# UCRajkumar/ecSeg

Measured on AMD Instinct MI355X. Metric: DAPI images/sec (1392x1040, 4-class metaseg), higher is better.
Workload: dtype f32; 1 GPU; BASELINE configs[1] + post-process: 16 synthetic 1040x1392 uint8 DAPI images per GPU per step, 35 tiles of 256x256 each, canonical U-Net base 64 (96.2 GFLOP/patch, seeded random weights) -> stitch/uint8-quantise/argmax -> meta_inference -> ecDNA count; unet_base=64, patches_per_image=35, parallelism=image-parallel x1, all-gather of 128-B records, allgather=none (1 rank)

## Files before the change

ecseg_amd/build.py:

```python
import os
import subprocess
import sys

HERE = os.path.dirname(os.path.abspath(__file__))
CSRC = os.path.join(HERE, 'csrc')
LIB = os.path.join(HERE, 'libecseg_hip.so')
SOURCES = ['api.hip', 'filter_layout.hip', 'model_load.hip', 'plan_run.hip', 'segment.hip', 'drivers.hip', 'unet_kernels.hip', 'layer_kernels.hip', 'wino4_kernel.hip', 'wino4s_kernel.hip', 'wino4r_kernel.hip', 'convs_kernel.hip', 'wino16_kernel.hip', 'post_kernels.hip', 'interseg_kernels.hip', 'fishdist_kernels.hip', 'fishspot_kernels.hip', 'host_codec.cpp', 'host_io.cpp', 'comm.hip']
EXTRA_FLAGS = {'wino4_kernel.hip': ['-fno-slp-vectorize'], 'wino4s_kernel.hip': ['-fno-slp-vectorize'], 'wino4r_kernel.hip': ['-fno-slp-vectorize']}
HEADERS = [os.path.join(CSRC, f) for f in ('common.h', 'ctx.h', 'device_util.h', 'wino4_consts.inc', 'wino4_region.inc', 'wino4_combine.inc', 'wino4_head.inc')] + \
    [os.path.join(HERE, '..', 'include', 'ecseg_hip.h')]


def source_hash():
    import hashlib
    h = hashlib.sha256()
    names = sorted(f for f in os.listdir(CSRC) if f.endswith(('.hip', '.h', '.inc')))
    for f in names:
        h.update(f.encode() + b'\0')
        with open(os.path.join(CSRC, f), 'rb') as fh:
            h.update(fh.read())
    return h.hexdigest()


def _hipcc():
    for c in (os.environ.get('HIPCC'), '/opt/rocm/bin/hipcc', 'hipcc'):
        if c and (os.path.isabs(c) and os.path.exists(c) or not os.path.isabs(c)):
            return c
    return 'hipcc'


def needs_build():
    if not os.path.exists(LIB):
        return True
    t = os.path.getmtime(LIB)
    deps = [os.path.join(CSRC, s) for s in SOURCES] + HEADERS
    return any(os.path.getmtime(d) > t for d in deps if os.path.exists(d))


def build(force=False, verbose=True):
    if not force and not needs_build():
        return LIB
    objs = []
    procs = []
    for s in SOURCES:
        obj = os.path.join(CSRC, os.path.splitext(s)[0] + '.o')
        cmd = [_hipcc(), '-O3', '-std=c++17', '--offload-arch=gfx950', '-fPIC', '-Wall', '-Wno-unused-function'] + \
            EXTRA_FLAGS.get(s, []) + ['-c', os.path.join(CSRC, s), '-o', obj]
        if verbose:
            print(' '.join(cmd), flush=True)
        procs.append((subprocess.Popen(cmd), cmd))
        objs.append(obj)
    for p, cmd in procs:
        if p.wait() != 0:
            raise RuntimeError('hipcc failed: ' + ' '.join(cmd))
    cmd = [_hipcc(), '--offload-arch=gfx950', '-shared', '-fPIC', '-o', LIB] + objs + ['-lz', '-ldl']
    if verbose:
        print(' '.join(cmd), flush=True)
    subprocess.check_call(cmd)
    return LIB


if __name__ == '__main__':
    build(force='--force' in sys.argv)
    print(LIB)
```

ecseg_amd/csrc/api.hip:

```cpp
#include <cstdio>
#include <cstdlib>
#include "ctx.h"

namespace ecseg {

namespace { std::string g_create_error; }

int fail(ecseg_ctx* h, int code, const std::string& msg) {
    if (h) h->err = msg; else g_create_error = msg;
    return code;
}
int fail_hip(ecseg_ctx* h, hipError_t e, const char* what) {
    return fail(h, ECSEG_E_HIP, std::string(what) + ": " + hipGetErrorString(e));
}

int check_model(ecseg_ctx* h) {
    if (!h) return ECSEG_E_INVALID;
    if (!h->has_model) return fail(h, ECSEG_E_NOMODEL, "no model loaded (call ecseg_model_load first)");
    return ECSEG_OK;
}

}

using namespace ecseg;

extern "C" {

int ecseg_abi_version(void) { return ECSEG_ABI_VERSION; }

int ecseg_create(ecseg_ctx** out, int device_id) {
    if (!out) return fail(nullptr, ECSEG_E_INVALID, "out is NULL");
    *out = nullptr;
    int ndev = 0;
    hipError_t e = hipGetDeviceCount(&ndev);
    if (e != hipSuccess || ndev <= 0) return fail(nullptr, ECSEG_E_HIP, std::string("no HIP device: ") + hipGetErrorString(e));
    if (device_id < 0 || device_id >= ndev) return fail(nullptr, ECSEG_E_INVALID, "device_id out of range");
    if ((e = hipSetDevice(device_id)) != hipSuccess) return fail_hip(nullptr, e, "hipSetDevice");
    if (!getenv("ECSEG_SPIN_WAIT") || atoi(getenv("ECSEG_SPIN_WAIT")) == 0) {
        if (hipSetDeviceFlags(hipDeviceScheduleBlockingSync) != hipSuccess) (void)hipGetLastError();
    }
    ecseg_ctx* h = new ecseg_ctx();
    h->device = device_id;
    hipDeviceProp_t prop;
    if (hipGetDeviceProperties(&prop, device_id) == hipSuccess) {
        snprintf(h->devname, sizeof(h->devname), "%s (%s)", prop.name, prop.gcnArchName);
    }
    if ((e = hipStreamCreateWithFlags(&h->stream, hipStreamNonBlocking)) != hipSuccess) {
        delete h;
        return fail_hip(nullptr, e, "hipStreamCreate");
    }
    if ((e = hipStreamCreateWithFlags(&h->stream2, hipStreamNonBlocking)) != hipSuccess) {
        (void)hipStreamDestroy(h->stream);
        delete h;
        return fail_hip(nullptr, e, "hipStreamCreate");
    }
    for (auto& ev : h->ev) (void)hipEventCreate(&ev);
    if (hipMalloc(reinterpret_cast<void**>(&h->zero_page), 1024) == hipSuccess) (void)hipMemset(h->zero_page, 0, 1024);
    else h->zero_page = nullptr;
    *out = h;
    return ECSEG_OK;
}

void ecseg_destroy(ecseg_ctx* h) {
    if (!h) return;
    (void)hipSetDevice(h->device);
    (void)hipStreamSynchronize(h->stream);
    (void)hipStreamSynchronize(h->stream2);
    free_model(h);
    if (h->zero_page) (void)hipFree(h->zero_page);
    { DevMem dying(std::move(static_cast<DevMem&>(*h))); }
    for (auto& ev : h->ev) if (ev) (void)hipEventDestroy(ev);
    if (h->ev_block) (void)hipEventDestroy(h->ev_block);
    if (h->stream_in) { (void)hipStreamSynchronize(h->stream_in); (void)hipStreamDestroy(h->stream_in); }
    if (h->ev_pre) (void)hipEventDestroy(h->ev_pre);
    for (hipEvent_t e : h->prof_events) (void)hipEventDestroy(e);
    for (hipEvent_t e : h->grp_events) (void)hipEventDestroy(e);
    for (hipEvent_t e : h->lane_events) (void)hipEventDestroy(e);
    for (hipStream_t ls : h->lane_streams) { (void)hipStreamSynchronize(ls); (void)hipStreamDestroy(ls); }
    (void)hipStreamDestroy(h->stream2);
    (void)hipStreamDestroy(h->stream);
    delete h;
}

const char* ecseg_last_error(ecseg_ctx* h) { return h ? h->err.c_str() : g_create_error.c_str(); }

int ecseg_device_name(ecseg_ctx* h, char* buf, int buflen) {
    if (!h || !buf || buflen <= 0) return ECSEG_E_INVALID;
    snprintf(buf, buflen, "%s", h->devname);
    return ECSEG_OK;
}

void* ecseg_stream(ecseg_ctx* h) { return h ? (void*)h->stream : nullptr; }

int ecseg_set_images_per_group(ecseg_ctx* h, int n) {
    if (!h || n < 0) return ECSEG_E_INVALID;
    h->images_per_group = n;
    return ECSEG_OK;
}

int ecseg_set_option(ecseg_ctx* h, const char* key, int value) {
    if (!h || !key) return ECSEG_E_INVALID;
    const std::string k(key);
    if (k == "overlap_post") h->overlap_post = value != 0;
    else if (k == "blocking_wait") h->blocking_wait = value != 0;
    else if (k == "fuse_pool") h->fuse_pool = value != 0;
    else if (k == "fuse_head") h->fuse_head = value != 0;
    else if (k == "wino_resident") h->wino_resident = value != 0;
    else if (k == "wino16") h->wino16 = value != 0;
    else if (k == "fuse_first") h->fuse_first = value != 0;
    else if (k == "wino4_split") h->wino4_split = value != 0;
    else if (k == "crop") h->crop = value != 0;
    else if (k == "winograd") {
        h->use_winograd = value < 0 ? 0 : value > 3 ? 3 : (int)value;
        return ensure_split_images(h);
    }
    else if (k == "post_chunk" && value >= 1) h->post_chunk = value;
    else if (k == "images_per_group" && value >= 0) h->images_per_group = value;
    else if (k == "crop_mask") h->crop_mask = value != 0;
    else if (k == "unet_lanes" && value >= 0 && value <= 8) h->unet_lanes = value;
    else if (k == "lane_auto_windows" && value >= 0) h->lane_auto_windows = value;
    else return fail(h, ECSEG_E_INVALID, "unknown option or bad value: " + k);
    return ECSEG_OK;
}

int ecseg_host_alloc(ecseg_ctx* h, size_t bytes, void** out) {
    if (!h || !out) return ECSEG_E_INVALID;
    *out = nullptr;
    if (bytes == 0) return ECSEG_OK;
    if (hipSetDevice(h->device) != hipSuccess) { (void)hipGetLastError(); return ECSEG_E_HIP; }
    const hipError_t e = hipHostMalloc(out, bytes, hipHostMallocPortable);
    if (e != hipSuccess) { (void)hipGetLastError(); *out = nullptr; return e == hipErrorOutOfMemory ? ECSEG_E_NOMEM : ECSEG_E_HIP; }
    return ECSEG_OK;
}

int ecseg_host_free(ecseg_ctx* h, void* p) {
    if (!h) return ECSEG_E_INVALID;
    if (!p) return ECSEG_OK;
    if (hipSetDevice(h->device) != hipSuccess || hipHostFree(p) != hipSuccess) { (void)hipGetLastError(); return ECSEG_E_HIP; }
    return ECSEG_OK;
}

int ecseg_get_timings(ecseg_ctx* h, float* ms_out) {
    if (!h || !ms_out) return ECSEG_E_INVALID;
    for (int k = 0; k < ECSEG_T_N; ++k) ms_out[k] = h->stage_ms[k];
    return ECSEG_OK;
}

int ecseg_set_kernel_profiling(ecseg_ctx* h, int enabled) {
    if (!h) return ECSEG_E_INVALID;
    h->profile_kernels = enabled != 0;
    return ECSEG_OK;
}

int ecseg_get_conv_profile(ecseg_ctx* h, double* total_ms, int64_t* launches, double* flops) {
    if (!h) return ECSEG_E_INVALID;
    if (total_ms) *total_ms = h->last_conv_ms;
    if (launches) *launches = h->last_conv_launches;
    if (flops) *flops = h->last_conv_flops;
    return ECSEG_OK;
}

int ecseg_debug_peek(ecseg_ctx* h, float* out, int n) {
#ifdef ECSEG_DIAG
    if (!h || !out || n < 0 || n > 240 || !h->zero_page) return ECSEG_E_INVALID;
    HIP_TRY(h, hipSetDevice(h->device));
    HIP_TRY(h, hipMemcpy(out, h->zero_page + 16, (size_t)n * sizeof(float), hipMemcpyDeviceToHost));
    return ECSEG_OK;
#else
    (void)out; (void)n;
    return fail(h, ECSEG_E_UNSUPPORTED, "ecseg_debug_peek: the shipped library carries no diagnostic kernels (build with -DECSEG_DIAG)");
#endif
}

int ecseg_get_conv_launch_profile(ecseg_ctx* h, int max_records, int32_t* op_index, int32_t* kind, float* ms, double* flops,
                                  double* executed_flops) {
    if (!h || max_records < 0) return ECSEG_E_INVALID;
    const int n = (int)std::min<size_t>(h->prof_recs.size(), (size_t)max_records);
    for (int k = 0; k < n; ++k) {
        const ecseg_ctx::ProfRec& r = h->prof_recs[k];
        if (op_index) op_index[k] = r.op;
        if (kind) kind[k] = r.kind;
        if (ms) ms[k] = r.ms;
        if (flops) flops[k] = r.flops;
        if (executed_flops) executed_flops[k] = r.exec_flops;
    }
    return n;
}

int ecseg_get_conv_executed_flops(ecseg_ctx* h, double* flops) {
    if (!h || !flops) return ECSEG_E_INVALID;
    *flops = h->last_conv_exec_flops;
    return ECSEG_OK;
}

}
```

ecseg_amd/csrc/common.h:

```cpp
#pragma once
#include <hip/hip_runtime.h>
#include <stdint.h>

#include "../../include/ecseg_hip.h"

namespace ecseg {

struct TView {
    float* p;
    int h, w, c, cs;
};

struct ConvParams {
    TView in, out;
    const float* wt;
    const float* bias;
    int n;
    int R, S;
    int pad_top, pad_left;
    int act;
    float alpha;
    int cin_chunks;
    int coutp;
    int convt;
    int kT, crop_top, crop_left;
    int convt_ext;
    int phase_a, phase_b;
    int tap_zero_mask;
    int stride;
    const float* zero;
    TView pool;
    const float* head_w; const float* head_b; TView head_out; int head_k, head_act, head_only;
    const int32_t* lut; int lut_len, per_image;
    const int32_t* in_box; int box_first;
    int force_tw;
    int resident;
    int w4_split;
    const float* first_w; const float* first_b; int first_act; float first_alpha;
    long wt_chunk_stride, wt_tap_stride;
};

#ifndef ECSEG_W4_PA
#define ECSEG_W4_PA 0.625
#define ECSEG_W4_PB 1.5
#endif
constexpr double W4_PA = ECSEG_W4_PA, W4_PB = ECSEG_W4_PB;

inline long wt_chunk_pitch(int np_total) { return (long)2 * np_total * 4 + 32; }
inline long wt_tap_pitch(int np_total, int chunks) { return wt_chunk_pitch(np_total) * chunks + 96; }

hipError_t launch_conv_mfma(const ConvParams& p, hipStream_t s);
bool       conv_mfma_supported(const ConvParams& p);
int        conv_mfma_ntile(int cout);
hipError_t launch_conv_wino(const ConvParams& p, hipStream_t s);
int        conv_wino_ntile(int cout);
hipError_t launch_conv_wino16(const ConvParams& p, hipStream_t s);
bool       conv_wino16_supported(const ConvParams& p);
bool       conv_wino16_first_supported(const ConvParams& p);
hipError_t launch_conv_wino4(const ConvParams& p, hipStream_t s);
bool       conv_wino4_supported(const ConvParams& p);
bool       conv_wino4_span_ok(const ConvParams& p, int windows);
hipError_t launch_conv_wino4r(const ConvParams& p, hipStream_t s);
bool       conv_wino4r_supported(const ConvParams& p);
hipError_t launch_conv_wino4s(const ConvParams& p, hipStream_t s);
bool       conv_wino4s_supported(const ConvParams& p);
size_t     wino4s_image_bytes(int cin, int cout);
hipError_t launch_wino4s_filter(const float* wt_wino4, void* dst, int cin, int cout, hipStream_t s);
hipError_t launch_convs(const ConvParams& p, hipStream_t s);
bool       convs_supported(const ConvParams& p);
size_t     convs_image_bytes(int cin, int np);
hipError_t launch_convs_filter(const float* wt_fp32, void* dst, int cin, int np, hipStream_t s);

hipError_t launch_conv_small_cin(const TView& in, const TView& out, const float* w_hwio, const float* bias, int n,
                                 int R, int S, int pad_top, int pad_left, int act, float alpha, hipStream_t s);
hipError_t launch_conv_head(const TView& in, const TView& out, const float* w_io, const float* bias, int n, int act,
                            float alpha, hipStream_t s);
hipError_t launch_conv_generic(const TView& in, const TView& out, const float* w_hwio, const float* bias, int n,
                               int R, int S, int stride, int pad_top, int pad_left, int act, float alpha, hipStream_t s);
hipError_t launch_convt_generic(const TView& in, const TView& out, const float* w_hwoi, const float* bias, int n,
                                int R, int S, int stride, int crop_top, int crop_left, int act, float alpha,
                                hipStream_t s);
hipError_t launch_maxpool(const TView& in, const TView& out, int n, int kh, int kw, int stride, int mode, hipStream_t s);
hipError_t launch_global_pool(const TView& in, const TView& out, int n, int mode, hipStream_t s);
hipError_t launch_upsample(const TView& in, const TView& out, int n, int factor, int mode, hipStream_t s);
hipError_t launch_affine(const TView& in, const TView& out, const float* scale, const float* shift, int n, int act,
                         float alpha, hipStream_t s);
hipError_t launch_add(const TView& a, const TView& b, const TView& out, int n, int act, float alpha, hipStream_t s);
hipError_t launch_copy(const TView& in, const TView& out, int n, int off_y, int off_x, hipStream_t s);
hipError_t launch_softmax(const TView& in, const TView& out, int n, hipStream_t s);
hipError_t launch_u8_to_f32(const uint8_t* in, float* out, size_t count, hipStream_t s);

hipError_t launch_conv_mfma_tap(const ConvParams& p, int dilation, hipStream_t s);
bool       conv_mfma_tap_supported(const ConvParams& p);
hipError_t launch_conv_generic_dil(const TView& in, const TView& out, const float* w_hwio, const float* bias, int n, int R, int S,
                                   int stride, int stride_x, int dilation, int dilation_x, int pad_top, int pad_left, int act, float alpha,
                                   hipStream_t s);
hipError_t launch_dwconv(const TView& in, const TView& out, const float* w, const float* bias, int n, int kh, int kw, int stride,
                         int dilation, int pad_top, int pad_left, int mult, int act, float alpha, hipStream_t s);
hipError_t launch_binary(const TView& a, const TView& b, const TView& out, int n, int mode, int act, float alpha, hipStream_t s);
hipError_t launch_prelu(const TView& in, const TView& out, const float* slope, int n, int per_element, hipStream_t s);
hipError_t launch_layernorm(const TView& in, const TView& out, const float* gamma, const float* beta, int n, float eps, hipStream_t s);
hipError_t launch_pool_pad(const TView& in, const TView& out, int n, int kh, int kw, int stride, int pad_top, int pad_left, int mode,
                           hipStream_t s);
hipError_t launch_tile_patches(const uint8_t* gray, int n_img, int H, int W, const int32_t* pos_yx, int n_pos,
                               float* out, hipStream_t s);

hipError_t launch_stitch_argmax(const float* probs, int prob_cs, const int32_t* src_map, int n_img, int n_pos,
                                int H, int W, uint8_t* labels, hipStream_t s, int32_t* tie_risk = nullptr, int32_t* tie_shards = nullptr);
hipError_t launch_stitch_probs(const float* probs, int prob_cs, const int32_t* src_map, int n_img, int n_pos,
                               int H, int W, float* out, hipStream_t s);

struct PostWorkspace {
    int32_t* L;
    uint32_t* area;
    unsigned long long* sumy;
    unsigned long long* sumx;
    uint32_t* flag;
    uint8_t* tmpA;
    uint8_t* tmpB;
    int32_t* list;
    int32_t* g;
    uint8_t* tile_any;
    uint32_t* own_bits;
    double* binned;
    int32_t* binstart;
    size_t binned_cap;
    int cap_img;
    size_t cap_px;
};
enum { G_STRIDE = 32, G_SHARDS = 16 };
enum { G_SLOTS = 6 };
enum { NUCLEUS_BIN_EXTENT = 32768 };

hipError_t run_meta_inference(PostWorkspace& ws, uint8_t* img, int n_img, int H, int W, int32_t* n_ec_dev,
                              hipStream_t s);
hipError_t run_count_cc(PostWorkspace& ws, const uint8_t* mask, int n_img, int H, int W, int32_t* n_dev,
                        long long* px_dev, hipStream_t s);
hipError_t run_ccl_labels(PostWorkspace& ws, const uint8_t* mask, int n_img, int H, int W, int conn,
                          int32_t* labels_dev, hipStream_t s);
hipError_t run_count_coloc(PostWorkspace& ws, const uint8_t* ob1, const uint8_t* ob2, int n_img, int H, int W,
                           int32_t* n_dev, hipStream_t s);
hipError_t run_count_hsr(PostWorkspace& ws, const uint8_t* chrom, const uint8_t* fish, int n_img, int H, int W,
                         int thr, int32_t* n_dev, hipStream_t s);
hipError_t run_overlay(PostWorkspace& ws, const uint8_t* labels, const uint8_t* rgb, int n_img, int H, int W, int C,
                       int sens, int hsr_thr, long long* out_dev, hipStream_t s);
hipError_t launch_u16_to_u8(const uint16_t* in, uint8_t* out, size_t count, hipStream_t s);
hipError_t run_preprocess(const void* img, int n_img, int H, int W, int C, int bps, uint8_t* gray, int32_t* inverted,
                          uint32_t* hist_ws, hipStream_t s);

struct RegionBufs { int32_t* rid; int32_t* blk; int32_t* misc; unsigned long long* acc; int32_t* bb; int64_t* rec; int cap; };
hipError_t run_nuclei_regions(const uint8_t* seg, const uint8_t* img, int H, int W, int img_w, int C, int ch0, int32_t* labels,
                              const RegionBufs& b, hipStream_t s);
hipError_t run_nucleus_crops(const int32_t* labels, const uint8_t* img, int W, int img_w, int C, const int32_t* desc, int n,
                             const int order[3], uint8_t* out, int32_t* chmax, hipStream_t s);

struct FishDistBufs { int32_t* rid; int32_t* par; int32_t* blk; int32_t* misc; int2* flist; int2* clist; unsigned* acc; int32_t* val;
                      int32_t* off; int32_t* cur; int64_t* rec; unsigned long long* pbest; int32_t* proots; };
int fishdist_slices(int n);
hipError_t run_fishdist_cells(const int32_t* labels, int H, int W, const FishDistBufs& b, hipStream_t s);
hipError_t run_fishdist_records(int32_t* labels, const uint8_t* lsq, int H, int W, int C, int fi, int ci, int n, const FishDistBufs& b,
                                hipStream_t s);

struct FishSpotBufs { int32_t* rid; int32_t* mx; uint8_t* thr; uint8_t* bnd; int32_t* par; int32_t* sz; unsigned long long* acc;
                      unsigned* cnt; int32_t* val; int64_t* rec; };
hipError_t run_fishspot(int32_t* labels, const uint8_t* img, int H, int W, int C, int np, const int ch[3], const double* wts, int K,
                        double normal_thr, const double ithr[3], int min_cc, int line_t, int n, const FishSpotBufs& b, hipStream_t s);

}
```

ecseg_amd/csrc/ctx.h:

```cpp
#pragma once
#include <algorithm>
#include <array>
#include <map>
#include <string>
#include <utility>
#include <vector>

#include "common.h"

namespace ecseg {

int fail(ecseg_ctx* h, int code, const std::string& msg);
int fail_hip(ecseg_ctx* h, hipError_t e, const char* what);
#define HIP_TRY(h, call) do { hipError_t _e = (call); if (_e != hipSuccess) return fail_hip((h), _e, #call); } while (0)

template <typename T>
struct DevBuf {
    T* p = nullptr;
    size_t cap = 0;
    DevBuf() = default;
    DevBuf(DevBuf&& o) noexcept { swap(o); }
    DevBuf(const DevBuf&) = delete;
    DevBuf& operator=(const DevBuf&) = delete;
    ~DevBuf() { if (p) (void)hipFree(p); }
    void swap(DevBuf& o) { std::swap(p, o.p); std::swap(cap, o.cap); }
    operator T*() const { return p; }
    int ensure(ecseg_ctx* h, size_t need_elems) {
        if (need_elems <= cap && p) return ECSEG_OK;
        if (p) { hipError_t e = hipFree(p); p = nullptr; cap = 0; if (e != hipSuccess) return fail_hip(h, e, "hipFree"); }
        if (need_elems == 0) need_elems = 1;
        hipError_t e = hipMalloc(reinterpret_cast<void**>(&p), need_elems * sizeof(T));
        if (e != hipSuccess) { p = nullptr; return fail(h, ECSEG_E_NOMEM, std::string("hipMalloc: ") + hipGetErrorString(e)); }
        cap = need_elems;
        return ECSEG_OK;
    }
};

struct OpRt {
    ecseg_op_desc d;
    int path;
    float* wt = nullptr;
    float* wt_wino = nullptr;
    float* wt_wino4 = nullptr;
    float* wt_wino16 = nullptr;
    void* wt_split1 = nullptr;
    int s1_cin = 0, s1_np = 0;
    void* wt_wino4s = nullptr;
    int w4_cin = 0, w4_cout = 0;
    int coutp_wino = 0;
    float* bias = nullptr;
    float* head_w4 = nullptr;
    float* head_b4 = nullptr;
    bool crop_ok = false;
    std::string crop_code;
    float* scale = nullptr;
    float* shift = nullptr;
    int cin_chunks = 0, coutp = 0;
    int subpixel = 0;
    float* ph_wt[4] = {nullptr, nullptr, nullptr, nullptr};
    int ph_R[4] = {0, 0, 0, 0}, ph_S[4] = {0, 0, 0, 0}, ph_pt[4] = {0, 0, 0, 0}, ph_pl[4] = {0, 0, 0, 0};
    double flops = 0.0;
};
enum { PATH_MFMA = 1, PATH_SMALL_CIN = 2, PATH_HEAD = 3, PATH_GENERIC = 4, PATH_OTHER = 5, PATH_TAP = 6  };

struct CropLut {
    DevBuf<int32_t> dev; int len = 0; int size = 0; std::vector<int> start;
};
struct StitchPlan {
    int n_pos = 0;
    DevBuf<int32_t> pos_dev;
    DevBuf<int32_t> map_dev;
    std::vector<int> box;
    std::map<std::string, CropLut> luts;
    std::map<std::string, DevBuf<int32_t>> boxes;
};

struct LaneSpec { int w0, cnt; hipStream_t s; };

void free_post_workspace(PostWorkspace& w);
struct OwnedPostWorkspace : PostWorkspace {
    OwnedPostWorkspace() : PostWorkspace{} {}
    OwnedPostWorkspace(OwnedPostWorkspace&& o) noexcept : PostWorkspace(o) { static_cast<PostWorkspace&>(o) = PostWorkspace{}; }
    ~OwnedPostWorkspace() { free_post_workspace(*this); }
};

struct DevMem {
    std::map<std::pair<int, int>, StitchPlan> stitch;
    DevBuf<uint8_t> d_gray, d_raw, d_post;
    DevBuf<int32_t> d_tie;
    DevBuf<int32_t> d_tie_sh;
    DevBuf<float> d_sprobs;
    DevBuf<uint8_t> d_aux8;
    DevBuf<uint8_t> d_pre;
    DevBuf<uint8_t> d_u8in;
    DevBuf<int32_t> d_i32;
    DevBuf<long long> d_i64;
    DevBuf<float> d_probs_in;
    DevBuf<uint32_t> d_hist;
    OwnedPostWorkspace ws;
    DevBuf<int32_t> d_iseg_lab, d_iseg_rid, d_iseg_blk, d_iseg_misc, d_iseg_bb, d_iseg_desc, d_iseg_max;
    DevBuf<uint8_t> d_iseg_img, d_iseg_crops;
    DevBuf<unsigned long long> d_iseg_acc;
    DevBuf<int64_t> d_iseg_rec;
    DevBuf<int32_t> d_fd_lab, d_fd_rid, d_fd_par, d_fd_blk, d_fd_misc, d_fd_val, d_fd_off, d_fd_cur, d_fd_proots;
    DevBuf<uint8_t> d_fd_lsq;
    DevBuf<int2> d_fd_flist, d_fd_clist;
    DevBuf<unsigned> d_fd_acc;
    DevBuf<int64_t> d_fd_rec;
    DevBuf<unsigned long long> d_fd_pbest;
    DevBuf<int32_t> d_fs_lab, d_fs_rid, d_fs_blk, d_fs_misc, d_fs_mx, d_fs_par, d_fs_sz, d_fs_val;
    DevBuf<uint8_t> d_fs_img, d_fs_thr, d_fs_bnd;
    DevBuf<double> d_fs_w;
    DevBuf<unsigned long long> d_fs_acc;
    DevBuf<unsigned> d_fs_cnt;
    DevBuf<int64_t> d_fs_rec;
};

}

struct ecseg_ctx : ecseg::DevMem {
    int device = 0;
    hipStream_t stream = nullptr;
    hipStream_t stream2 = nullptr;
    std::vector<hipStream_t> lane_streams;
    std::vector<hipEvent_t> lane_events;
    int unet_lanes = 0;
    int lane_auto_windows = 70;
    bool lanes_ok = false;
    std::string err;
    char devname[256] = {0};

    bool has_model = false;
    std::vector<ecseg_tensor_desc> tensors;
    std::vector<ecseg::OpRt> ops;
    int n_buffers = 0;
    std::vector<size_t> buf_floats;
    std::vector<float*> bufs;
    int cap_patches = 0;
    std::vector<float*> dev_allocs;
    float* zero_page = nullptr;
    int input_tensor = -1, output_tensor = -1;
    std::vector<int> consumers;
    double flops_per_patch = 0.0, mfma_flops_per_patch = 0.0;

    int images_per_group = 0;
    const void* pre_host = nullptr; size_t pre_bytes = 0;
    const void* next_host = nullptr; size_t next_bytes = 0;
    hipStream_t stream_in = nullptr;
    hipEvent_t ev_pre = nullptr;
    int iseg_H = 0, iseg_W = 0, iseg_img_w = 0, iseg_C = 0, iseg_n = -1;
    int post_chunk = 64;
    int overlap_post = 0;
    int blocking_wait = 1;
    hipEvent_t ev_block = nullptr;
    int fuse_pool = 1;
    int crop = 1;
    int crop_mask = 1;
    int fuse_head = 1;
    int use_winograd = 2;
    int wino4_split = 1;
    int wino16 = 1;
    int wino_resident = 1;
    int fuse_first = 1;

    hipEvent_t ev[ECSEG_T_N + 1] = {};
    float stage_ms[ECSEG_T_N] = {};
    bool profile_kernels = false;
    std::vector<hipEvent_t> prof_events;
    std::vector<hipEvent_t> grp_events;
    size_t prof_used = 0;
    double prof_flops = 0.0, prof_exec_flops = 0.0;
    struct ProfRec { int op; int kind; double flops, exec_flops; float ms; };
    std::vector<ProfRec> prof_recs;
    double last_conv_ms = 0.0; long long last_conv_launches = 0; double last_conv_flops = 0.0, last_conv_exec_flops = 0.0;
};

namespace ecseg {

inline TView view_of(const ecseg_ctx* h, int t) {
    const ecseg_tensor_desc& d = h->tensors[t];
    TView v;
    v.p = h->bufs[d.buffer] + d.c_offset;
    v.h = d.h; v.w = d.w; v.c = d.c; v.cs = d.c_stride;
    return v;
}

inline float stage_elapsed(hipEvent_t a, hipEvent_t b) {
    float t = 0.f;
    return hipEventElapsedTime(&t, a, b) == hipSuccess ? t : 0.f;
}

inline void drop_sent_ahead(ecseg_ctx* h) {
    h->next_host = nullptr; h->next_bytes = 0;
    h->pre_host = nullptr; h->pre_bytes = 0;
}

int check_model(ecseg_ctx* h);

std::vector<float> relayout_conv(const float* w, int R, int S, int cin, int cout, int chunks, int np);
std::vector<float> relayout_wino16(const std::vector<float>& u, int cin, int cout);
std::vector<float> winograd_filter(const float* w, int cin, int cout);
std::vector<float> winograd4_filter(const float* w, int cin, int cout);
std::vector<float> relayout_convt(const float* w, int kT, int cin, int cout, int chunks, int coutp);
std::vector<float> relayout_convt_subpixel(const float* w, int k, int cin, int cout, int chunks, int coutp);
struct PhaseFilter { std::vector<float> hwio; int R, S, pt, pl; };
std::array<PhaseFilter, 4> convt_phase_filters(const float* w, int k, int cin, int cout, int crop_top, int crop_left);

void free_model(ecseg_ctx* h);
int ensure_split_images(ecseg_ctx* h);

int ensure_patches(ecseg_ctx* h, int n);
int windows_per_group(const ecseg_ctx* h);
int run_plan(ecseg_ctx* h, int n_all, StitchPlan* crop = nullptr, const std::vector<LaneSpec>* lanes = nullptr);
void prof_begin(ecseg_ctx* h);
void prof_end(ecseg_ctx* h);

int get_stitch(ecseg_ctx* h, int H, int W, StitchPlan** out);
int ensure_post(ecseg_ctx* h, int n_img, size_t px);

}
```

ecseg_amd/csrc/plan_run.hip:

```cpp
#include "ctx.h"

namespace ecseg {

int ensure_patches(ecseg_ctx* h, int n) {
    if (n <= h->cap_patches) return ECSEG_OK;
    for (float*& p : h->bufs) { if (p) (void)hipFree(p); p = nullptr; }
    h->bufs.assign(h->n_buffers, nullptr);
    h->cap_patches = 0;
    for (int b = 0; b < h->n_buffers; ++b) {
        const size_t bytes = std::max<size_t>(h->buf_floats[b], 4) * (size_t)n * sizeof(float);
        hipError_t e = hipMalloc(reinterpret_cast<void**>(&h->bufs[b]), bytes);
        if (e != hipSuccess) return fail(h, ECSEG_E_NOMEM, std::string("hipMalloc(activations): ") + hipGetErrorString(e));
    }
    h->cap_patches = n;
    return ECSEG_OK;
}

int windows_per_group(const ecseg_ctx* h) {
    if (h->images_per_group > 0) return h->images_per_group * 35;
    size_t per_window = 0;
    for (size_t f : h->buf_floats) per_window += std::max<size_t>(f, 4) * sizeof(float);
    const size_t budget = (size_t)48 << 30;
    size_t img = per_window ? budget / (per_window * 35) : 16;
    int g = 16;
// ... 130 lines not shown

int run_plan_op(ecseg_ctx* h, size_t& oi, int n_all, StitchPlan* crop, const LaneSpec* ls) {
    hipStream_t s = ls ? ls->s : h->stream;
    const bool lane = ls != nullptr;
    const int n = lane ? ls->cnt : n_all;
    const int w0 = lane ? ls->w0 : 0, cnt = n;
    const bool part = lane && crop && (w0 % crop->n_pos != 0 || cnt % crop->n_pos != 0);
    const int wbase = part ? (w0 / crop->n_pos) * crop->n_pos : w0;
    if (part && w0 + cnt > wbase + crop->n_pos) return fail(h, ECSEG_E_INVALID, "window lane crosses an image boundary");
    auto at = [&](int t, bool rebase = false) {
        if (t < 0) return TView{};
        TView v = view_of(h, t);
        if (!lane) return v;
        const ecseg_tensor_desc& td = h->tensors[t];
        const ptrdiff_t hwc = (ptrdiff_t)v.h * v.w * v.cs;
        const bool io = t == h->input_tensor || t == h->output_tensor;
        ptrdiff_t off = io ? (ptrdiff_t)w0 * hwc : (ptrdiff_t)w0 * (ptrdiff_t)std::max<size_t>(h->buf_floats[td.buffer], 4);
        if (rebase) off -= (ptrdiff_t)(w0 - wbase) * hwc;
        v.p += off;
        return v;
    };
    const OpRt* first = nullptr;
    if (first_layer_fusable(h, oi, crop != nullptr)) first = &h->ops[oi++];
    {
        const OpRt& o = h->ops[oi];
        const ecseg_op_desc& d = o.d;
        const TView in = first ? at(first->d.in0) : at(d.in0), out = at(d.out);
        hipError_t e = hipSuccess;
        switch (d.op) {
            case ECSEG_OP_CONV:
            case ECSEG_OP_CONVT: {
                const bool softmax = d.act == ECSEG_ACT_SOFTMAX;
                const int act = (softmax && o.path != PATH_HEAD) ? ECSEG_ACT_LINEAR : d.act;
                if (o.path == PATH_MFMA) {
                    const size_t oi_first = oi;
                    ConvParams p = conv_params(h, o, in, out, n, act);
                    if (d.op == ECSEG_OP_CONV && d.kh == 1 && d.kw == 1 && in.h == 1 && in.w == 1 && out.h == 1 && out.w == 1) {
                        p.in.w = n; p.out.w = n; p.n = 1;
                    }
                    bool rebased = false;
                    auto use_lut = [&](const CropLut* cl) {
                        p.lut = cl->dev; p.lut_len = cl->len; p.per_image = crop->n_pos;
                        if (part) {
                            const int a = cl->start[w0 - wbase], b = cl->start[w0 - wbase + cnt];
                            p.lut = cl->dev + a; p.lut_len = b - a; p.n = crop->n_pos;
                            rebased = true;
                            p.box_first = 0;
                            p.in = at(d.in0, true); p.out = at(d.out, true);
                        }
                    };
                    hipEvent_t* ev = h->profile_kernels ? prof_pair(h) : nullptr;
                    if (ev) (void)hipEventRecord(ev[0], s);
                    double computed = 1.0;
                    const bool act_core_ok = act <= ECSEG_ACT_ELU && !(act == ECSEG_ACT_ELU && d.alpha != 1.f);
                    if (first) {
                        p.first_w = first->wt; p.first_b = first->bias; p.first_act = first->d.act; p.first_alpha = first->d.alpha;
                    }
                    const bool wino4 = !first && h->use_winograd >= 2 && o.wt_wino4 && act_core_ok && conv_wino4_supported(p);
                    const bool wino = !wino4 && h->use_winograd && o.wt_wino && out.h >= 4 && out.w >= 8;
                    bool w16 = false, split1 = false;
                    const bool crop_on = crop && h->crop && o.crop_ok && (part || n % crop->n_pos == 0);
                    if (crop_on && h->crop_mask && d.op == ECSEG_OP_CONV && d.kh == 3 && d.kw == 3 && (wino4 || wino)) {
                        p.in_box = get_crop_box(crop, o.crop_code + "d");
                        p.per_image = crop->n_pos;
                        p.box_first = part ? w0 - wbase : 0;
                    }
                    auto fuse_following_pool = [&]() {
                        if (oi + 1 >= h->ops.size()) return;
                        const ecseg_op_desc& nx = h->ops[oi + 1].d;
                        const TView po = nx.op == ECSEG_OP_MAXPOOL ? at(nx.out, rebased) : TView{};
                        if (nx.op == ECSEG_OP_MAXPOOL && nx.mode == 0  && nx.in0 == d.out && nx.kh == 2 && nx.kw == 2 && nx.stride == 2 &&
                            h->fuse_pool && !softmax && po.h * 2 == out.h && po.w * 2 == out.w && po.c == out.c && po.cs % 4 == 0 &&
                            reinterpret_cast<uintptr_t>(po.p) % 16 == 0 &&
                            h->tensors[nx.out].buffer != h->tensors[d.in0].buffer && h->tensors[nx.out].buffer != h->tensors[d.out].buffer) {
                            p.pool = po;
                            ++oi;
                        }
                    };
                    auto fuse_following_head = [&](int channels) {
                        if (p.pool.p != nullptr || oi + 1 >= h->ops.size() || !h->fuse_head || out.c != channels || softmax) return;
                        const OpRt& hx = h->ops[oi + 1];
                        const ecseg_tensor_desc& td = h->tensors[d.out];
                        if (hx.d.op == ECSEG_OP_CONV && hx.path == PATH_HEAD && hx.head_w4 && hx.d.in0 == d.out && hx.d.act <= ECSEG_ACT_TANH &&
                            hx.d.act != ECSEG_ACT_LEAKY  &&
                            h->consumers[d.out] == 1 && d.out != h->output_tensor && td.c_stride == td.c && td.c_offset == 0 &&
                            h->tensors[hx.d.out].buffer != h->tensors[d.in0].buffer &&
                            h->tensors[hx.d.out].buffer != td.buffer) {
                            p.head_w = hx.head_w4; p.head_b = hx.head_b4; p.head_out = at(hx.d.out, rebased);
                            p.head_k = p.head_out.c; p.head_act = hx.d.act; p.head_only = 1;
                            ++oi;
                        }
                    };
                    const bool wino4s = wino4 && h->use_winograd >= 3 && o.wt_wino4s && conv_wino4s_supported(p);
                    if (wino4) {
                        p.wt = wino4s ? reinterpret_cast<const float*>(o.wt_wino4s) : o.wt_wino4; p.coutp = out.c; p.w4_split = h->wino4_split;
                        if (crop_on) {
                            const CropLut* cl = get_crop_lut(crop, o.crop_code);
                            if (cl->len > 0 && out.h == cl->size && out.w == cl->size && conv_wino4_span_ok(p, crop->n_pos)) {
                                use_lut(cl);
                                computed = (double)cl->len / ((double)crop->n_pos * (out.h / 16) * (out.w / 16));
                            }
                        }
                        fuse_following_pool();
                        fuse_following_head(64);
                        e = wino4s ? launch_conv_wino4s(p, s) : conv_wino4r_supported(p) ? launch_conv_wino4r(p, s) : launch_conv_wino4(p, s);
                    } else if (wino && h->wino16 && o.wt_wino16 && act_core_ok && (first ? conv_wino16_first_supported(p) : conv_wino16_supported(p))) {
                        w16 = true;
                        p.wt = o.wt_wino16;
                        if (crop_on) {
                            const CropLut* cl = get_crop_lut(crop, o.crop_code, 16, 32);
                            if (cl->len > 0 && out.h == cl->size && out.w == cl->size) {
                                use_lut(cl);
                                computed = (double)cl->len / ((double)crop->n_pos * (out.h / 16) * (out.w / 32));
                            }
                        }
                        fuse_following_pool();
                        fuse_following_head(out.c);
                        e = launch_conv_wino16(p, s);
                    } else if (wino) {
                        p.wt = o.wt_wino; p.coutp = o.coutp_wino;
                        p.wt_chunk_stride = wt_chunk_pitch(o.coutp_wino); p.wt_tap_stride = wt_tap_pitch(o.coutp_wino, o.cin_chunks);
                        p.resident = h->wino_resident;
                        if (out.c % 4 == 0) fuse_following_pool();
                        e = launch_conv_wino(p, s);
                    } else {
                        if (crop_on && p.convt && in.h == in.w) {
                            const CropLut* a = get_crop_lut(crop, o.crop_code, 4, 32);
                            const CropLut* b = get_crop_lut(crop, o.crop_code, 8, 16);
                            const CropLut* cl = nullptr; int tw = 0;
                            if (a->len > 0 && a->size == in.h && in.w >= 32 && (b->len == 0 || b->size != in.h || a->len <= b->len)) { cl = a; tw = 32; }
                            else if (b->len > 0 && b->size == in.h) { cl = b; tw = 16; }
                            if (cl) {
                                use_lut(cl); p.force_tw = tw;
                                const int th = 128 / tw;
                                computed = (double)cl->len / ((double)crop->n_pos * ((in.h + th - 1) / th) * ((in.w + tw - 1) / tw));
                            }
                        }
                        if (o.subpixel && o.ph_wt[0] != nullptr) {
                            p.tap_zero_mask = 0;
                            p.crop_top = 0; p.crop_left = 0;
                            p.convt_ext = ((out.h + 1) / 2 > in.h || (out.w + 1) / 2 > in.w) ? 1 : 0;
                            for (int ph = 0; ph < 4 && e == hipSuccess; ++ph) {
                                p.wt = o.ph_wt[ph]; p.R = o.ph_R[ph]; p.S = o.ph_S[ph]; p.pad_top = o.ph_pt[ph]; p.pad_left = o.ph_pl[ph];
                                p.phase_a = ph >> 1; p.phase_b = ph & 1;
                                p.convt = 2;
                                p.wt_chunk_stride = wt_chunk_pitch(o.coutp);
                                p.wt_tap_stride = wt_tap_pitch(o.coutp, o.cin_chunks);
                                e = launch_conv_mfma(p, s);
                            }
                        } else if (h->use_winograd >= 3 && o.wt_split1 != nullptr && p.convt == 1 && convs_supported(p)) {
                            p.wt = reinterpret_cast<const float*>(o.wt_split1);
                            split1 = true;
                            e = launch_convs(p, s);
                        } else {
                            e = launch_conv_mfma(p, s);
                        }
                    }
                    if (first && !w16 && e == hipSuccess) e = hipErrorInvalidValue;
                    if (ev) {
                        const double fl1 = first ? first->flops * n : 0.0;
                        const double ex = o.flops * n * computed * (wino4 ? 0.25 : wino ? 16.0 / 36.0 : (o.subpixel && o.ph_wt[0] == nullptr) ? (16.0 - __builtin_popcount((unsigned)p.tap_zero_mask)) / (d.kh * d.kw) : 1.0);
                        const bool res = wino && p.resident && p.coutp == 32 && p.cin_chunks <= 4;
                        prof_record(h, ev, s, (int)oi_first, (split1 ? 6 : wino4s ? 5 : wino4 ? 2 : w16 ? 4 : res ? 3 : wino ? 1 : 0) | (p.pool.p != nullptr ? 0x100 : 0) |
                                    (p.head_w != nullptr ? 0x200 : 0) | (first ? 0x400 : 0), o.flops * n + fl1, ex + fl1 * 12.0 / 9.0);
                    }
                } else if (o.path == PATH_TAP) {
                    const ConvParams p = conv_params(h, o, in, out, n, act);
                    hipEvent_t* ev = h->profile_kernels ? prof_pair(h) : nullptr;
                    if (ev) (void)hipEventRecord(ev[0], s);
                    e = launch_conv_mfma_tap(p, d.dilation, s);
                    if (ev) prof_record(h, ev, s, (int)oi, 0, o.flops * n, o.flops * n);
                } else if (o.path == PATH_SMALL_CIN) {
                    e = launch_conv_small_cin(in, out, o.wt, o.bias, n, d.kh, d.kw, d.pad_top, d.pad_left, act, d.alpha, s);
                } else if (o.path == PATH_HEAD) {
                    e = launch_conv_head(in, out, o.wt, o.bias, n, d.act, d.alpha, s);
                } else if (d.op == ECSEG_OP_CONV) {
                    if (d.dilation > 1 || (d.mode & 0xffff))
                        e = launch_conv_generic_dil(in, out, o.wt, o.bias, n, d.kh, d.kw, d.stride, (d.mode & 0xff) ? (d.mode & 0xff) : d.stride, d.dilation > 1 ? d.dilation : 1,
                                                    ((d.mode >> 8) & 0xff) ? ((d.mode >> 8) & 0xff) : (d.dilation > 1 ? d.dilation : 1), d.pad_top, d.pad_left, act, d.alpha, s);
                    else e = launch_conv_generic(in, out, o.wt, o.bias, n, d.kh, d.kw, d.stride, d.pad_top, d.pad_left, act, d.alpha, s);
                } else {
                    e = launch_convt_generic(in, out, o.wt, o.bias, n, d.kh, d.kw, d.stride, d.pad_top, d.pad_left, act, d.alpha, s);
                }
                if (e == hipSuccess && softmax && o.path != PATH_HEAD) e = launch_softmax(out, out, n, s);
                break;
            }
            case ECSEG_OP_MAXPOOL:
                if (d.pad_top || d.pad_left || (out.h - 1) * d.stride + d.kh > in.h || (out.w - 1) * d.stride + d.kw > in.w)
                    e = launch_pool_pad(in, out, n, d.kh, d.kw, d.stride, d.pad_top, d.pad_left, d.mode, s);
                else e = launch_maxpool(in, out, n, d.kh, d.kw, d.stride, d.mode, s);
                break;
            case ECSEG_OP_DWCONV: {
                const bool softmax = d.act == ECSEG_ACT_SOFTMAX;
                e = launch_dwconv(in, out, o.wt, o.bias, n, d.kh, d.kw, d.stride, d.dilation, d.pad_top, d.pad_left, d.mode,
                                  softmax ? ECSEG_ACT_LINEAR : d.act, d.alpha, s);
                if (e == hipSuccess && softmax) e = launch_softmax(out, out, n, s);
                break;
            }
            case ECSEG_OP_PRELU: e = launch_prelu(in, out, o.wt, n, d.mode, s); break;
            case ECSEG_OP_LAYERNORM: e = launch_layernorm(in, out, o.scale, o.shift, n, d.alpha, s); break;
            case ECSEG_OP_GLOBALPOOL: e = launch_global_pool(in, out, n, d.mode, s); break;
            case ECSEG_OP_UPSAMPLE: e = launch_upsample(in, out, n, d.stride, d.mode, s); break;
            case ECSEG_OP_AFFINE:
                if (d.act == ECSEG_ACT_SOFTMAX) {
                    e = launch_affine(in, out, o.scale, o.shift, n, ECSEG_ACT_LINEAR, d.alpha, s);
                    if (e == hipSuccess) e = launch_softmax(out, out, n, s);
                } else {
                    e = launch_affine(in, out, o.scale, o.shift, n, d.act, d.alpha, s);
                }
                break;
            case ECSEG_OP_ACT:
                if (d.act == ECSEG_ACT_SOFTMAX) e = launch_softmax(in, out, n, s);
                else e = launch_affine(in, out, nullptr, nullptr, n, d.act, d.alpha, s);
                break;
            case ECSEG_OP_ADD: {
                const TView b = at(d.in1);
                const bool same = in.h == out.h && in.w == out.w && in.c == out.c && b.h == out.h && b.w == out.w && b.c == out.c;
                if (d.mode == ECSEG_BIN_ADD && same && d.act != ECSEG_ACT_SOFTMAX) e = launch_add(in, b, out, n, d.act, d.alpha, s);
                else {
                    e = launch_binary(in, b, out, n, d.mode, d.act == ECSEG_ACT_SOFTMAX ? ECSEG_ACT_LINEAR : d.act, d.alpha, s);
                    if (e == hipSuccess && d.act == ECSEG_ACT_SOFTMAX) e = launch_softmax(out, out, n, s);
                }
                break;
            }
            case ECSEG_OP_COPY: e = launch_copy(in, out, n, d.pad_top, d.pad_left, s); break;
            default: return fail(h, ECSEG_E_INVALID, "unknown op in plan");
        }
        if (e != hipSuccess) return fail_hip(h, e, "plan kernel launch");
    }
    return ECSEG_OK;
}

}

int run_plan(ecseg_ctx* h, int n_all, StitchPlan* crop, const std::vector<LaneSpec>* lanes) {
    for (size_t oi = 0; oi < h->ops.size(); ++oi) {
        int rc;
        if (!lanes || lanes->empty()) {
            if ((rc = run_plan_op(h, oi, n_all, crop, nullptr))) return rc;
        } else {
            size_t last = oi;
            for (const LaneSpec& l : *lanes) {
                size_t o2 = oi;
                if (l.cnt > 0 && (rc = run_plan_op(h, o2, n_all, crop, &l))) return rc;
                if (l.cnt > 0) last = o2;
            }
            oi = last;
        }
    }
    return ECSEG_OK;
}

void prof_begin(ecseg_ctx* h) { h->prof_used = 0; h->prof_flops = 0.0; h->prof_exec_flops = 0.0; h->prof_recs.clear(); }
void prof_end(ecseg_ctx* h) {
    double ms = 0.0;
    for (size_t k = 0; k + 1 < h->prof_used; k += 2) {
        float t = 0.f;
        if (hipEventElapsedTime(&t, h->prof_events[k], h->prof_events[k + 1]) == hipSuccess) ms += t;
        if (k / 2 < h->prof_recs.size()) h->prof_recs[k / 2].ms = t;
    }
    h->last_conv_ms = ms; h->last_conv_launches = (long long)(h->prof_used / 2); h->last_conv_flops = h->prof_flops;
    h->last_conv_exec_flops = h->prof_exec_flops;
}

}

using namespace ecseg;

static int forward_host(ecseg_ctx* h, const void* patches, bool is_f32, int n, float* out) {
    if (h) drop_sent_ahead(h);
    int rc = check_model(h);
    if (rc) return rc;
    if (n < 0 || (n > 0 && (!patches || !out))) return fail(h, ECSEG_E_INVALID, "forward_patches: bad arguments");
    if (n == 0) return ECSEG_OK;
    HIP_TRY(h, hipSetDevice(h->device));
    const ecseg_tensor_desc& ti = h->tensors[h->input_tensor];
    const ecseg_tensor_desc& to = h->tensors[h->output_tensor];
    if (ti.c_stride != ti.c || ti.c_offset != 0) return fail(h, ECSEG_E_INVALID, "input tensor must be compact");
    const size_t in_per = (size_t)ti.h * ti.w * ti.c, out_per = (size_t)to.h * to.w * to.c;
    const int chunk = std::max(1, windows_per_group(h));
    if ((rc = ensure_patches(h, std::min(n, chunk)))) return rc;
    if (!is_f32 && (rc = h->d_u8in.ensure(h, in_per * std::min(n, chunk)))) return rc;
    hipStream_t s = h->stream;
    prof_begin(h);
    for (int i0 = 0; i0 < n; i0 += chunk) {
        const int ni = std::min(chunk, n - i0);
        if (is_f32) {
            HIP_TRY(h, hipMemcpyAsync(view_of(h, h->input_tensor).p, static_cast<const float*>(patches) + (size_t)i0 * in_per,
                                      in_per * ni * sizeof(float), hipMemcpyHostToDevice, s));
        } else {
            HIP_TRY(h, hipMemcpyAsync(h->d_u8in, static_cast<const uint8_t*>(patches) + (size_t)i0 * in_per, in_per * ni, hipMemcpyHostToDevice, s));
            HIP_TRY(h, launch_u8_to_f32(h->d_u8in, view_of(h, h->input_tensor).p, in_per * ni, s));
        }
        if ((rc = run_plan(h, ni))) return rc;
        const TView ov = view_of(h, h->output_tensor);
        HIP_TRY(h, hipMemcpy2DAsync(out + (size_t)i0 * out_per, (size_t)to.c * sizeof(float), ov.p, (size_t)ov.cs * sizeof(float),
                                    (size_t)to.c * sizeof(float), (size_t)to.h * to.w * ni, hipMemcpyDeviceToHost, s));
        HIP_TRY(h, hipStreamSynchronize(s));
    }
    prof_end(h);
    return ECSEG_OK;
}

extern "C" {

int ecseg_forward_patches(ecseg_ctx* h, const uint8_t* patches, int n, float* out) { return forward_host(h, patches, false, n, out); }
// ... 18 lines not shown
```

Before: 110.1 images/s.

## Add dedicated GEMM kernel for 2x2 stride-2 transposed convolutions

```diff
diff --git a/ecseg_amd/build.py b/ecseg_amd/build.py
--- a/ecseg_amd/build.py
+++ b/ecseg_amd/build.py
@@ -5,7 +5,7 @@
 HERE = os.path.dirname(os.path.abspath(__file__))
 CSRC = os.path.join(HERE, 'csrc')
 LIB = os.path.join(HERE, 'libecseg_hip.so')
-SOURCES = ['api.hip', 'filter_layout.hip', 'model_load.hip', 'plan_run.hip', 'segment.hip', 'drivers.hip', 'unet_kernels.hip', 'layer_kernels.hip', 'wino4_kernel.hip', 'wino4s_kernel.hip', 'wino4r_kernel.hip', 'convs_kernel.hip', 'wino16_kernel.hip', 'post_kernels.hip', 'interseg_kernels.hip', 'fishdist_kernels.hip', 'fishspot_kernels.hip', 'host_codec.cpp', 'host_io.cpp', 'comm.hip']
+SOURCES = ['api.hip', 'filter_layout.hip', 'model_load.hip', 'plan_run.hip', 'segment.hip', 'drivers.hip', 'unet_kernels.hip', 'layer_kernels.hip', 'wino4_kernel.hip', 'wino4s_kernel.hip', 'wino4r_kernel.hip', 'convs_kernel.hip', 'convt_gemm_kernel.hip', 'wino16_kernel.hip', 'post_kernels.hip', 'interseg_kernels.hip', 'fishdist_kernels.hip', 'fishspot_kernels.hip', 'host_codec.cpp', 'host_io.cpp', 'comm.hip']
 EXTRA_FLAGS = {'wino4_kernel.hip': ['-fno-slp-vectorize'], 'wino4s_kernel.hip': ['-fno-slp-vectorize'], 'wino4r_kernel.hip': ['-fno-slp-vectorize']}
 HEADERS = [os.path.join(CSRC, f) for f in ('common.h', 'ctx.h', 'device_util.h', 'wino4_consts.inc', 'wino4_region.inc', 'wino4_combine.inc', 'wino4_head.inc')] + \
     [os.path.join(HERE, '..', 'include', 'ecseg_hip.h')]
diff --git a/ecseg_amd/csrc/api.hip b/ecseg_amd/csrc/api.hip
--- a/ecseg_amd/csrc/api.hip
+++ b/ecseg_amd/csrc/api.hip
@@ -109,6 +109,7 @@
     else if (k == "wino16") h->wino16 = value != 0;
     else if (k == "fuse_first") h->fuse_first = value != 0;
     else if (k == "wino4_split") h->wino4_split = value != 0;
+    else if (k == "up2_gemm") h->up2_gemm = value != 0;
     else if (k == "crop") h->crop = value != 0;
     else if (k == "winograd") {
         h->use_winograd = value < 0 ? 0 : value > 3 ? 3 : (int)value;
diff --git a/ecseg_amd/csrc/common.h b/ecseg_amd/csrc/common.h
--- a/ecseg_amd/csrc/common.h
+++ b/ecseg_amd/csrc/common.h
@@ -70,6 +70,8 @@
 bool       convs_supported(const ConvParams& p);
 size_t     convs_image_bytes(int cin, int np);
 hipError_t launch_convs_filter(const float* wt_fp32, void* dst, int cin, int np, hipStream_t s);
+hipError_t launch_conv_up2(const ConvParams& p, hipStream_t s);
+bool       conv_up2_supported(const ConvParams& p);
 
 hipError_t launch_conv_small_cin(const TView& in, const TView& out, const float* w_hwio, const float* bias, int n,
                                  int R, int S, int pad_top, int pad_left, int act, float alpha, hipStream_t s);
diff --git a/ecseg_amd/csrc/convt_gemm_kernel.hip b/ecseg_amd/csrc/convt_gemm_kernel.hip
--- /dev/null
+++ b/ecseg_amd/csrc/convt_gemm_kernel.hip
@@ -0,0 +1,188 @@
+#include "common.h"
+#include "device_util.h"
+
+namespace ecseg {
+
+namespace {
+typedef __attribute__((address_space(3))) void* lptr_t;
+constexpr int UP2_BM = 128, UP2_BN = 256, UP2_NT = UP2_BN / 32;
+constexpr int UP2_A_SLOTS = 2 * 2 * UP2_BM, UP2_B_SLOTS = 2 * 2 * UP2_BN, UP2_STAGE = UP2_A_SLOTS + UP2_B_SLOTS;
+constexpr int UP2_NBUF = 3;
+constexpr int UP2_DMAS = 6;
+}
+
+#define UP2_WAIT(n) asm volatile("s_waitcnt vmcnt(" #n ")" ::: "memory")
+#define UP2_BARRIER() asm volatile("s_waitcnt lgkmcnt(0)\n\ts_barrier" ::: "memory")
+
+template <int PD>
+__global__ __launch_bounds__(256, 2) void conv_up2_kernel(ConvParams p, int tiles_x, int tiles_y, int nblk_n, int np_total, int tw_shift) {
+    extern __shared__ __attribute__((aligned(16))) char smem[];
+    f32x4* S = reinterpret_cast<f32x4*>(smem);
+    const unsigned lds_base = (unsigned)(size_t)(lptr_t)smem;
+
+    const int tid = threadIdx.x, lane = tid & 63;
+    const int wave = __builtin_amdgcn_readfirstlane(tid >> 6);
+    const int li = lane & 31, lh = lane >> 5;
+    const int TW = 1 << tw_shift, TH = UP2_BM >> tw_shift;
+
+    unsigned bid = xcd_remap(blockIdx.x, gridDim.x);
+    const int nb = bid % nblk_n; bid /= nblk_n;
+    int tx0, ty0, img;
+    if (p.lut != nullptr) {
+        const int i = bid / p.lut_len, v = p.lut[bid - i * p.lut_len];
+        img = i * p.per_image + (v >> 16); ty0 = ((v >> 8) & 255) * 4; tx0 = (v & 255) * 4;
+    } else {
+        tx0 = (bid % tiles_x) * TW; bid /= tiles_x;
+        ty0 = (bid % tiles_y) * TH; bid /= tiles_y;
+        img = bid;
+    }
+    const int n0 = nb * UP2_BN;
+    const int Hin = p.in.h, Win = p.in.w, Cin = p.in.c;
+
+    const int kc_w = wave >> 1, h_w = wave & 1;
+    const float* a_pix[2];
+#pragma unroll
+    for (int j = 0; j < 2; ++j) {
+        const int pix = j * 64 + lane;
+        const int iy = ty0 - p.pad_top + (pix >> tw_shift), ix = tx0 - p.pad_left + (pix & (TW - 1));
+        a_pix[j] = (iy >= 0 && iy < Hin && ix >= 0 && ix < Win) ? p.in.p + ((size_t)img * Hin * Win + (size_t)iy * Win + ix) * p.in.cs : nullptr;
+    }
+    const float* b_lane = p.wt + ((size_t)h_w * np_total + n0 + lane) * 4;
+    const size_t chunk_stride = (size_t)p.wt_chunk_stride;
+    const int nstages = (p.cin_chunks + 1) / 2;
+
+    auto dma_stage = [&](int st) __attribute__((always_inline)) {
+        const int c = min(st * 2 + kc_w, p.cin_chunks - 1), ch = c * 8 + h_w * 4;
+        const unsigned dst = lds_base + (unsigned)((st % UP2_NBUF) * UP2_STAGE) * 16u;
+        const unsigned dst_a = dst + (unsigned)((kc_w * 2 + h_w) * UP2_BM) * 16u;
+        const unsigned dst_b = dst + (unsigned)(UP2_A_SLOTS + (kc_w * 2 + h_w) * UP2_BN) * 16u;
+        const float* a0 = (a_pix[0] != nullptr && ch < Cin) ? a_pix[0] + ch : p.zero;
+        const float* a1 = (a_pix[1] != nullptr && ch < Cin) ? a_pix[1] + ch : p.zero;
+        const float* b = b_lane + (size_t)c * chunk_stride;
+        unsigned keep;
+        asm volatile("s_mov_b32 %0, m0\n\ts_mov_b32 m0, %2\n\ts_nop 0\n\tglobal_load_lds_dwordx4 %1, off\n\ts_mov_b32 m0, %0"
+                     : "=&s"(keep) : "v"(a0), "s"(dst_a) : "memory");
+        asm volatile("s_mov_b32 %0, m0\n\ts_mov_b32 m0, %2\n\ts_nop 0\n\tglobal_load_lds_dwordx4 %1, off\n\ts_mov_b32 m0, %0"
+                     : "=&s"(keep) : "v"(a1), "s"(dst_a + 1024u) : "memory");
+        asm volatile("s_mov_b32 %0, m0\n\ts_mov_b32 m0, %2\n\ts_nop 0\n\t"
+                     "global_load_lds_dwordx4 %1, off\n\t"
+                     "global_load_lds_dwordx4 %1, off offset:1024\n\t"
+                     "global_load_lds_dwordx4 %1, off offset:2048\n\t"
+                     "global_load_lds_dwordx4 %1, off offset:3072\n\t"
+                     "s_mov_b32 m0, %0"
+                     : "=&s"(keep) : "v"(b), "s"(dst_b) : "memory");
+    };
+
+    f32x16 acc[UP2_NT];
+#pragma unroll
+    for (int nt = 0; nt < UP2_NT; ++nt)
+#pragma unroll
+        for (int e = 0; e < 16; ++e) acc[nt][e] = 0.f;
+
+    dma_stage(0);
+    if (nstages > 1) dma_stage(1);
+    for (int st = 0; st < nstages; ++st) {
+        if (st + 1 < nstages) UP2_WAIT(6); else UP2_WAIT(0);
+        UP2_BARRIER();
+        if (st + 2 < nstages) dma_stage(st + 2);
+        const f32x4* Ap = S + (st % UP2_NBUF) * UP2_STAGE + lh * UP2_BM + wave * 32 + li;
+        const f32x4* Bp = S + (st % UP2_NBUF) * UP2_STAGE + UP2_A_SLOTS + lh * UP2_BN + li;
+#pragma unroll
+        for (int kc = 0; kc < 2; ++kc) {
+            if (kc == 1 && st * 2 + 1 >= p.cin_chunks) break;
+            const f32x4 a = Ap[kc * 2 * UP2_BM];
+#pragma unroll
+            for (int nt = 0; nt < UP2_NT; ++nt) {
+                const f32x4 b = Bp[kc * 2 * UP2_BN + nt * 32];
+#pragma unroll
+                for (int e = 0; e < 4; ++e) acc[nt] = __builtin_amdgcn_mfma_f32_32x32x2f32(a[e], b[e], acc[nt], 0, 0, 0);
+            }
+        }
+    }
+    static_assert(UP2_DMAS == 6, "UP2_WAIT(6) above counts the DMAs of one stage");
+    __syncthreads();
+
+    const int Hout = p.out.h, Wout = p.out.w, Cout = p.out.c;
+    const int Ht = Hin + p.convt_ext, Wt = Win + p.convt_ext;
+    float* Xs = reinterpret_cast<float*>(smem) + wave * 2048;
+    const bool vec_ok = (p.out.cs % 4 == 0) && (Cout % 4 == 0) && ((reinterpret_cast<uintptr_t>(p.out.p) & 15) == 0);
+    const int quad = lane & 7;
+    auto finish = [&](int col, int row, f32x4 v) __attribute__((always_inline)) {
+        const int ab = col / p.coutp, co = col - ab * p.coutp;
+        const int oa = ab >> 1, ob = ab & 1;
+        f32x4 bv = {0.f, 0.f, 0.f, 0.f};
+        if (p.bias != nullptr) {
+#pragma unroll
+            for (int c = 0; c < 4; ++c) if (co + c < Cout) bv[c] = p.bias[co + c];
+        }
+        v = apply_act4(v + bv, p.act, p.alpha);
+        const int pix = wave * 32 + row;
+        const int tyy = ty0 + (pix >> tw_shift), txx = tx0 + (pix & (TW - 1));
+        const int oy = tyy * 2 + oa - p.crop_top, ox = txx * 2 + ob - p.crop_left;
+        if (tyy < Ht && txx < Wt && oy >= 0 && oy < Hout && ox >= 0 && ox < Wout) {
+            float* o = p.out.p + (((size_t)img * Hout + oy) * Wout + ox) * p.out.cs + co;
+            if (vec_ok && co + 3 < Cout) __builtin_nontemporal_store(v, reinterpret_cast<f32x4*>(o));
+            else {
+#pragma unroll
+                for (int c = 0; c < 4; ++c) if (co + c < Cout) o[c] = v[c];
+            }
+        }
+    };
+#pragma unroll
+    for (int nt = 0; nt < UP2_NT; ++nt) {
+        if constexpr (PD > 0) {
+            if ((nt / PD) & 1) continue;
+#pragma unroll
+            for (int e = 0; e < 16; ++e) {
+                Xs[((e & 3) + 8 * (e >> 2) + 4 * lh) * 32 + li] = acc[nt][e];
+                Xs[1024 + ((e & 3) + 8 * (e >> 2) + 4 * lh) * 32 + li] = acc[(nt + PD) % UP2_NT][e];
+            }
+            const int b = (lane >> 3) & 1;
+#pragma unroll
+            for (int r = 0; r < 8; ++r) {
+                const int row = (lane >> 4) + 4 * r;
+                finish(n0 + (nt + b * PD) * 32 + 4 * quad, row, *reinterpret_cast<const f32x4*>(Xs + b * 1024 + row * 32 + 4 * quad));
+            }
+        } else {
+#pragma unroll
+            for (int e = 0; e < 16; ++e) Xs[((e & 3) + 8 * (e >> 2) + 4 * lh) * 32 + li] = acc[nt][e];
+#pragma unroll
+            for (int r = 0; r < 4; ++r) {
+                const int row = (lane >> 3) + 8 * r;
+                finish(n0 + nt * 32 + 4 * quad, row, *reinterpret_cast<const f32x4*>(Xs + row * 32 + 4 * quad));
+            }
+        }
+    }
+}
+#undef UP2_WAIT
+#undef UP2_BARRIER
+
+bool conv_up2_supported(const ConvParams& p) {
+    const bool align_ok = (p.in.cs % 4 == 0) && (p.in.c % 4 == 0) && (((uintptr_t)p.in.p) % 16 == 0);
+    return p.convt == 1 && p.R == 1 && p.S == 1 && p.kT == 2 && p.stride <= 1 && p.phase_a == 0 && p.phase_b == 0 && align_ok &&
+           p.in.c >= 8 && p.out.c >= 16 && p.coutp > 0 && p.coutp % 64 == 0 && p.zero != nullptr;
+}
+
+hipError_t launch_conv_up2(const ConvParams& p, hipStream_t s) {
+    if (!conv_up2_supported(p)) return hipErrorInvalidValue;
+    const bool wide = p.force_tw ? p.force_tw == 32 : p.in.w >= 32;
+    const int tw_shift = wide ? 5 : 4, TW = 1 << tw_shift, TH = UP2_BM / TW;
+    const int ext_h = p.in.h + p.convt_ext, ext_w = p.in.w + p.convt_ext;
+    const int tiles_x = (ext_w + TW - 1) / TW, tiles_y = (ext_h + TH - 1) / TH;
+    const int np_total = 4 * p.coutp, nblk_n = np_total / UP2_BN;
+    const size_t grid = (p.lut != nullptr ? (size_t)(p.n / p.per_image) * p.lut_len : (size_t)p.n * tiles_x * tiles_y) * nblk_n;
+    if (grid == 0) return hipSuccess;
+    if (grid > 0x7fffffffull) return hipErrorInvalidValue;
+    const size_t lds = (size_t)UP2_NBUF * UP2_STAGE * 16;
+    const int v = p.coutp == 64 ? 1 : p.coutp == 128 ? 2 : 0;
+    void (*kern)(ConvParams, int, int, int, int, int) = v == 1 ? conv_up2_kernel<2> : v == 2 ? conv_up2_kernel<4> : conv_up2_kernel<0>;
+    static DeviceOnce attr_set[3];
+    const hipError_t ea = attr_set[v].run([&] {
+        return hipFuncSetAttribute(reinterpret_cast<const void*>(kern), hipFuncAttributeMaxDynamicSharedMemorySize, (int)lds);
+    });
+    if (ea != hipSuccess) return ea;
+    hipLaunchKernelGGL(kern, dim3((unsigned)grid), dim3(256), lds, s, p, tiles_x, tiles_y, nblk_n, np_total, tw_shift);
+    return hipGetLastError();
+}
+
+}
diff --git a/ecseg_amd/csrc/ctx.h b/ecseg_amd/csrc/ctx.h
--- a/ecseg_amd/csrc/ctx.h
+++ b/ecseg_amd/csrc/ctx.h
@@ -158,6 +158,7 @@
     int crop_mask = 1;
     int fuse_head = 1;
     int use_winograd = 2;
+    int up2_gemm = 1;
     int wino4_split = 1;
     int wino16 = 1;
     int wino_resident = 1;
diff --git a/ecseg_amd/csrc/plan_run.hip b/ecseg_amd/csrc/plan_run.hip
--- a/ecseg_amd/csrc/plan_run.hip
+++ b/ecseg_amd/csrc/plan_run.hip
@@ -306,6 +306,8 @@
                             p.wt = reinterpret_cast<const float*>(o.wt_split1);
                             split1 = true;
                             e = launch_convs(p, s);
+                        } else if (h->up2_gemm && conv_up2_supported(p)) {
+                            e = launch_conv_up2(p, s);
                         } else {
                             e = launch_conv_mfma(p, s);
                         }
```

Result: slower. 108.9 images/s (-1.1%).
